# glennhickey/teHmm

Measured on AMD Instinct MI355X. Metric: genome positions/sec (Viterbi+posterior), 35 states x 10 tracks, higher is better.
Workload: dtype f64

## Files before the change

### tehmm_amd/csrc/tehmm_aux.hip.h

```cpp
#pragma once
#include "tehmm_kernels.hip.h"

namespace tehmm {

__global__ __launch_bounds__(256) void k_segment_table(int64_t T, int K, const uint8_t *data, int64_t n_seg,
                                                       const int64_t *off, const uint8_t *is_gauss,
                                                       const double *mapback, uint8_t *out, double *means) {
  __shared__ unsigned hist[4][256];
  const int lane = threadIdx.x & 63, w = threadIdx.x >> 6;
  const int64_t nw = (int64_t)gridDim.x * 4;
  for (int64_t i = (int64_t)blockIdx.x * 4 + w; i < n_seg; i += nw) {
    const int64_t a = off[i], b = i + 1 < n_seg ? off[i + 1] : T;
    for (int k = 0; k < K; ++k) {
      if (is_gauss[k]) {
        if (lane == 0) {
          const double *mb = mapback + (int64_t)k * 256;
          double total = 0.0;
          for (int64_t x = a; x < b; ++x) total += mb[data[x * K + k]];
          means[i * K + k] = total / (double)(b - a);
          out[i * K + k] = data[a * K + k];
        }
        continue;
      }
      unsigned *h = hist[w];
// ... 256 lines not shown
      const int j = kq + 4 * s;
      double v = 0.0;
      if (s < KS && j < N) v = log_domain ? row[j] : (dead ? 0.0 : exp(row[j] - c));
      else if (s < KS && log_domain) v = -INFINITY;
      else if (s == KS) v = (log_domain || dead) ? 0.0 : c;
      o[kq * KSP + s] = v;
    }
  }
}
__global__ void k_pack_ptab_lds(int K, const int *rowbase, const int *rowcnt, const int *ldsbase, int lds_zero,
                                int zero_row, int ROW_D, int ROW_L, const double *ptab, double *ptab_lds) {
  const int k = blockIdx.x;
  int src, dst, cnt;
  if (k == K) { src = zero_row; dst = lds_zero; cnt = 1; }
  else { if (ldsbase[k] < 0) return; src = rowbase[k]; dst = ldsbase[k]; cnt = rowcnt[k]; }
  for (int i = threadIdx.x; i < cnt * ROW_L; i += blockDim.x) {
    const int r = i / ROW_L, c = i - r * ROW_L;
    ptab_lds[(int64_t)(dst + r) * ROW_L + c] = c < ROW_D ? ptab[(int64_t)(src + r) * ROW_D + c] : 0.0;
  }
}

__global__ void k_stats_logprob(int n, const int *ids, const double *fwd_lp, double *stats) {
  if (blockIdx.x == 0 && threadIdx.x == 0) {
    double s = 0.0;
    for (int i = 0; i < n; ++i) s += fwd_lp[ids[i]];
    stats[0] += s;
    stats[1] += (double)n;
  }
}

}
```

### tehmm_amd/csrc/tehmm_fused.hip.h

```cpp
#pragma once
#include "tehmm_lane.hip.h"

namespace tehmm {

template <int NT>
struct FusedGeom {
  static constexpr int KS = NT / 4;
  static constexpr int KSP = ((KS + 1) + 1) & ~1;
  static constexpr int RT = (NT + 15) / 16;
  static constexpr int SLICE_B = KSP * 8;
  static constexpr int ROW_D = 4 * KSP;
  static constexpr int ROW_D_LDS = 4 * KSP + 2;
};

#ifndef TEHMM_FUSED_2W
#define TEHMM_FUSED_2W 36
#endif
#define TEHMM_FUSED_BLKW 24
#ifndef TEHMM_FUSED_NSLOT_CAP
#define TEHMM_FUSED_NSLOT_CAP 64
#endif

struct FusedTab {
  const unsigned long long *rixx;
  const double *ptab;
  const double *ptab_lds;
  int FKW;
  int SB, NB;
  int K, n_glb;
  int lds_rows;
  double normalize;
};

template <int NT>
__device__ __forceinline__ void fused_load_lds(const double *lds, int row, int kq, double (&x)[FusedGeom<NT>::KSP]) {
  using G = FusedGeom<NT>;
  lds_cd2 *p = (lds_cd2 *)(size_t)((unsigned)(size_t)(__attribute__((address_space(3))) const double *)lds +
                                   (unsigned)(row * (G::ROW_D_LDS * 8) + kq * G::SLICE_B));
#pragma unroll
  for (int i = 0; i < G::KSP / 2; ++i) {
    const d2v v = p[i];
    x[2 * i] = v.x;
    x[2 * i + 1] = v.y;
  }
}
template <int NT>
__device__ __forceinline__ void fused_load_glb(const double *tab, int row, int kq, double (&x)[FusedGeom<NT>::KSP]) {
// ... 16 lines not shown
  const auto c = __builtin_amdgcn_permlane16_swap(lo1, lo1, false, false);
  const auto d = __builtin_amdgcn_permlane16_swap(hi1, hi1, false, false);
  return __hiloint2double((int)d[0], (int)c[0]) + __hiloint2double((int)d[1], (int)c[1]);
}
__device__ __forceinline__ double item_max4(double t) {
  const unsigned lo = __double2loint(t), hi = __double2hiint(t);
  const auto a = __builtin_amdgcn_permlane32_swap(lo, lo, false, false);
  const auto b = __builtin_amdgcn_permlane32_swap(hi, hi, false, false);
  const double t1 = fmax(__hiloint2double((int)b[0], (int)a[0]), __hiloint2double((int)b[1], (int)a[1]));
  const unsigned lo1 = __double2loint(t1), hi1 = __double2hiint(t1);
  const auto c = __builtin_amdgcn_permlane16_swap(lo1, lo1, false, false);
  const auto d = __builtin_amdgcn_permlane16_swap(hi1, hi1, false, false);
  return fmax(__hiloint2double((int)d[0], (int)c[0]), __hiloint2double((int)d[1], (int)c[1]));
}

typedef unsigned int fused_u4 __attribute__((ext_vector_type(4)));
struct IndexWindow {
  const fused_u4 *src;
  unsigned lds_base;
  int lane, dir, NB;
  int cur = -1;
  fused_u4 r0, r1, r2;
  bool inflight = false;

  __device__ __forceinline__ void request(int blk) {
    if (blk < 0 || blk >= NB) { inflight = false; return; }
    const fused_u4 *p = src + (int64_t)blk * 192 + lane * 3;
    r0 = p[0];
    r1 = p[1];
    r2 = p[2];
    inflight = true;
  }
  __device__ __forceinline__ void commit(int blk) {
    typedef __attribute__((address_space(3))) fused_u4 lds_u4;
    lds_u4 *d = (lds_u4 *)(size_t)(lds_base + (unsigned)((blk & 1) * 3072 + lane * 48));
    d[0] = r0;
    d[1] = r1;
    d[2] = r2;
    cur = blk;
  }
  __device__ __forceinline__ void start(int blk) {
    request(blk);
    commit(blk);
    request(blk + dir);
  }
  __device__ __forceinline__ void need(int blk) {
    if (blk != cur) {
      commit(blk);
      request(blk + dir);
    }
  }
  __device__ __forceinline__ unsigned word_addr(int blk, int r, int FKW, int w) const {
    return lds_base + (unsigned)((blk & 1) * 3072 + ((r * FKW + w) * 16 + (lane & 15)) * 8);
  }
};
__device__ __forceinline__ unsigned long long lds_read_u64(unsigned addr) {
  typedef __attribute__((address_space(3))) const unsigned long long lds_cu64;
  return *(lds_cu64 *)(size_t)addr;
}

template <int NT, bool LOGDOM>
struct EmisStream {
  using G = FusedGeom<NT>;
  static constexpr int NSLOT = G::KS < TEHMM_FUSED_NSLOT_CAP ? G::KS : TEHMM_FUSED_NSLOT_CAP;
  static constexpr int NGS = NSLOT > 1 ? 2 : 1;
  static constexpr int GF = NSLOT >= 8 ? 4 : NSLOT / 2;
  const FusedTab &ft;
  const double *lds;
  IndexWindow &win;
  const int kq;
  unsigned wbase = 0;
  double q[G::KS];
  double sc = 0.0;
  double xa[G::KSP];
  double xc[G::KSP];
  unsigned long long wcur = 0;

  __device__ __forceinline__ EmisStream(const FusedTab &ft_, const double *lds_, IndexWindow &win_, int kq_)
      : ft(ft_), lds(lds_), win(win_), kq(kq_) {}
  static __device__ __forceinline__ int entry(unsigned long long w, int i) { return (int)((w >> (16 * (i & 3))) & 0xffffull); }
  __device__ __forceinline__ unsigned long long word(int w) const { return lds_read_u64(wbase + (unsigned)w * 128u); }
  __device__ __forceinline__ void fold(const double (&x)[G::KSP]) {
#pragma unroll
    for (int s = 0; s < G::KS; ++s) q[s] = LOGDOM ? q[s] + x[s] : q[s] * x[s];
    if (!LOGDOM) sc += x[G::KS];
  }
  __device__ __forceinline__ void glb_request(int i) { fused_load_glb<NT>(ft.ptab, entry(word(i >> 2), i), kq, xa); }
  __device__ __forceinline__ void begin(int e) {
    const int blk = e / ft.SB, r = e - blk * ft.SB;
    win.need(blk);
    wbase = win.word_addr(blk, r, ft.FKW, 0);
#pragma unroll
    for (int s = 0; s < G::KS; ++s) q[s] = LOGDOM ? 0.0 : 1.0;
    sc = 0.0;
    glb_request(0);
    wcur = word(ft.n_glb >> 2);
  }
  __device__ __forceinline__ void slot(int k) {
    if (k >= NSLOT) return;
    const int il = ft.n_glb + k;
    if (k > 0) fold(xc);
    if (k == GF && NSLOT > 1) {
      fold(xa);
      glb_request(1);
    }
    fused_load_lds<NT>(lds, entry(wcur, il), kq, xc);
    if (k + 1 < NSLOT) wcur = word((il + 1) >> 2);
  }
  __device__ __forceinline__ void finish(int N, double (&qo)[G::KS], double &ms) {
    fold(xc);
    fold(xa);
    for (int i = NGS; i < ft.n_glb; ++i) {
      glb_request(i);
      fold(xa);
    }
    for (int il = ft.n_glb + NSLOT; il < ft.K; ++il) {
      fused_load_lds<NT>(lds, entry(word(il >> 2), il), kq, xc);
      fold(xc);
    }
    if (LOGDOM) {
      double m = -INFINITY;
#pragma unroll
      for (int s = 0; s < G::KS; ++s) {
        q[s] *= ft.normalize;
        m = fmax(m, kq + 4 * s < N ? q[s] : -INFINITY);
      }
      m = item_max4(m);
      const bool good = m > -1e20;
#pragma unroll
      for (int s = 0; s < G::KS; ++s) qo[s] = (good && kq + 4 * s < N) ? exp_nonpos(q[s] - m) : 0.0;
      ms = good ? m : 0.0;
    } else {
#pragma unroll
      for (int s = 0; s < G::KS; ++s) qo[s] = q[s];
      ms = sc;
    }
  }
};

template <int NT>
__host__ __device__ inline size_t fused_lds_bytes(int lds_rows, bool post_tiles) {
  return (size_t)lds_rows * FusedGeom<NT>::ROW_D_LDS * 8 + 4 * 2 * 3072 + (post_tiles ? 4 * (16 * NT * 8 + 128) : 0);
}
template <int NT>
__device__ __forceinline__ void fused_stage(const FusedTab &ft, double *lds) {
  const int n = ft.lds_rows * FusedGeom<NT>::ROW_D_LDS;
  for (int i = threadIdx.x; i < n; i += blockDim.x) lds[i] = ft.ptab_lds[i];
}

struct FusedOrder {
  int K, n_glb, FKW, KP, SB, NB, Wu;
  int zero_glb, zero_lds;
  unsigned char order[TEHMM_MAX_TRACKS];
  int base[TEHMM_MAX_TRACKS];
  int cnt[TEHMM_MAX_TRACKS];
};
__global__ __launch_bounds__(256) void k_fused_rowindex(IntervalTab iv, LaneGeom lg, FusedOrder fo, const uint8_t *obs,
                                                        unsigned long long *rixx) {
  const int E = fo.NB * fo.SB;
  const int64_t n = (int64_t)lg.n_groups * 4 * E * 16;
  const int per_blk = 16 * fo.SB;
  for (int64_t idx = blockIdx.x * (int64_t)blockDim.x + threadIdx.x; idx < n; idx += (int64_t)gridDim.x * blockDim.x) {
    const int64_t tb = idx / per_blk;
    const int rem = (int)(idx - tb * per_blk);
    const int i16 = rem / fo.SB;
    const int e = (int)(tb % fo.NB) * fo.SB + (rem - i16 * fo.SB);
    const int64_t tile = tb / fo.NB;
    const int64_t item = tile * 16 + i16;
    const bool valid = item < lg.n_items;
    const int id = valid ? lg.item_iv[item] : 0;
    const int64_t T = iv.len[id];
    int64_t t = (valid ? lg.item_t0[item] : 0) - fo.Wu + e;
    t = t < 0 ? 0 : (t >= T ? T - 1 : t);
    const uint8_t *orow = obs + (iv.pos0[id] + (T > 0 ? t : 0)) * fo.KP;
    const int blk = e / fo.SB, r = e - blk * fo.SB;
    unsigned long long *dst = rixx + ((tile * fo.NB + blk) * TEHMM_FUSED_BLKW + (int64_t)r * fo.FKW) * 16 + i16;
    for (int w = 0; w < fo.FKW; ++w) {
      unsigned long long word = 0;
      for (int b = 0; b < 4; ++b) {
        const int i = 4 * w + b;
        int v = 0;
        if (i < fo.K) {
          const int sym = orow[fo.order[i]];
          v = sym < fo.cnt[i] ? fo.base[i] + sym : (i < fo.n_glb ? fo.zero_glb : fo.zero_lds);
        }
        word |= (unsigned long long)(v & 0xffff) << (16 * b);
      }
      dst[(int64_t)w * 16] = word;
    }
  }
}

template <int NT, bool LOGDOM>
__global__ __launch_bounds__(256) __attribute__((amdgpu_waves_per_eu(NT <= TEHMM_FUSED_2W ? 2 : 1, NT <= TEHMM_FUSED_2W ? 2 : 1)))
void k_fused_fwd(IntervalTab iv, FusedTab ft, LaneGeom lg, int N, int CS, int Wu,
                 const double *__restrict__ tab , float *al32, double *chkf, double *pre,
                 double *end, double *slog32) {
  using G = FusedGeom<NT>;
  constexpr int KS = G::KS, RT = G::RT;
  extern __shared__ double fused_lds[];
  fused_stage<NT>(ft, fused_lds);
  __syncthreads();
  const int lane = threadIdx.x & 63;
  const int tile = blockIdx.x * 4 + (threadIdx.x >> 6);
  if (tile >= lg.n_groups * 4) return;
// ... 14 lines not shown
    for (int s = 0; s < KS; ++s) {
      const int j = 16 * rt + (lane & 15), k = 4 * s + kq;
      tf[rt][s] = (j < NT) ? tab[k * NT + j] : 0.0;
    }
  }
  double v[KS];
#pragma unroll
  for (int s = 0; s < KS; ++s) v[s] = (kq + 4 * s < N) ? 1.0 / (double)N : 0.0;
  double slog = 0.0;
  auto vec_out = [&](double *dst) {
    const int64_t po = ((((item >> 6) * NT) + kq) << 6) + (item & 63);
#pragma unroll
    for (int s = 0; s < KS; ++s) dst[po + ((int64_t)(4 * s) << 6)] = v[s];
  };
  const double qnan = __longlong_as_double(0x7ff8000000000000LL);
  IndexWindow win;
  win.src = (const fused_u4 *)ft.rixx + (int64_t)tile * ft.NB * 192;
  win.lds_base = (unsigned)(size_t)(__attribute__((address_space(3))) const double *)fused_lds +
                 (unsigned)(ft.lds_rows * G::ROW_D_LDS * 8 + (threadIdx.x >> 6) * 2 * 3072);
  win.lane = lane;
  win.dir = 1;
  win.NB = ft.NB;
  win.start(0);
  double q[KS], ms;
  EmisStream<NT, LOGDOM> es(ft, fused_lds, win, kq);
  es.begin(0);
#pragma unroll
  for (int k = 0; k < KS; ++k) es.slot(k);
  es.finish(N, q, ms);
  const int E1 = ft.NB * ft.SB - 1;
  es.begin(min(1, E1));
  {
    float2 *ar = (float2 *)al32 + al32_index<NT>(lg, item, 0, kq) / 2;
#pragma unroll
    for (int p = 0; p < (KS + 1) / 2; ++p) ar[(int64_t)p * 64] = make_float2(0.f, 0.f);
  }
#ifdef TEHMM_STAMPS
// ... 104 lines not shown
    }
  }
  double v[KS];
#pragma unroll
  for (int s = 0; s < KS; ++s) v[s] = 0.0;
  const int64_t prow0 = (iv.out0[id] + t0) * N;
  auto vec_out = [&](double *dst) {
    const int64_t po = ((((item >> 6) * NT) + kq) << 6) + (item & 63);
#pragma unroll
    for (int s = 0; s < KS; ++s) dst[po + ((int64_t)(4 * s) << 6)] = v[s];
  };
  const double eps = 1.1920928955078125e-07;
  const double inv_epsden = 1.0 / (1.0 + (double)N * eps);
  const double qnan = __longlong_as_double(0x7ff8000000000000LL);
  const int top = L + wu - 1;
  IndexWindow win;
  win.src = (const fused_u4 *)ft.rixx + (int64_t)tile * ft.NB * 192;
  win.lds_base = (unsigned)(size_t)(__attribute__((address_space(3))) const double *)fused_lds +
                 (unsigned)(ft.lds_rows * G::ROW_D_LDS * 8 + (threadIdx.x >> 6) * 2 * 3072);
  win.lane = lane;
  win.dir = -1;
  win.NB = ft.NB;
  win.start((L + 2 * Wu - 1) / ft.SB);
  typedef __attribute__((address_space(3))) double lds_f64;
  typedef __attribute__((address_space(3))) long long lds_i64;
  const unsigned ptile = (unsigned)(size_t)(__attribute__((address_space(3))) const double *)fused_lds +
                         (unsigned)(ft.lds_rows * G::ROW_D_LDS * 8 + 4 * 2 * 3072 + (threadIdx.x >> 6) * (16 * NT * 8 + 128));
  const unsigned pinfo = ptile + 16 * NT * 8;
  if (!ESTEP && kq == 0) *(lds_i64 *)(size_t)(pinfo + (lane & 15) * 8) = run ? (long long)prow0 : -1ll;
  double q[KS], ms;
  EmisStream<NT, LOGDOM> es(ft, fused_lds, win, kq);
  es.begin(L + 2 * Wu - 1);
#pragma unroll
  for (int k = 0; k < KS; ++k) es.slot(k);
  es.finish(N, q, ms);
  es.begin(max(L + 2 * Wu - 2, 0));
#ifdef TEHMM_STAMPS
  unsigned long long stq[4] = {0, 0, 0, 0}, stt = stamp_now();
#define FST(i) do { const unsigned long long n_ = stamp_now(); stq[i] += n_ - stt; stt = n_; } while (0)
#else
#define FST(i)
#endif
// ... 141 lines not shown
```

### tehmm_amd/csrc/tehmm_hip.hip

```cpp
#include <climits>
#include "tehmm_kernels.hip.h"
#include "tehmm_coop.hip.h"
#include "tehmm_lane.hip.h"
#include "tehmm_lane3.hip.h"
#include "tehmm_place.hip.h"
#include "tehmm_aux.hip.h"
#include "tehmm_fused.hip.h"
#include "tehmm_estep.hip.h"
#include "tehmm_wide_estep.hip.h"
#include "tehmm_wide.hip.h"
#include "tehmm_large.hip.h"

#include <algorithm>
#include <atomic>
#include <cmath>
#include <cstdio>
#include <cstdlib>
#include <cstring>
#include <mutex>
#include <numeric>
#include <string>
#include <thread>
#include <vector>

// ... 224 lines not shown
  double normalize = 1.0;
  DBuf<double> lt, ltT, A, AT, pi, tab, ltab;
  DBuf<double> ltG, AG, ATG;
  DBuf<float> ltP;
  DBuf<double> ptab, ptab_lds;
  DBuf<int> d_rowinfo;
  int KSP = 0;
  bool large = false;
  uint64_t uid = 0;
  uint64_t version = 0;
  bool ptab_log = false;
  int rowbase[TEHMM_MAX_TRACKS];
  int rowcnt[TEHMM_MAX_TRACKS];
  int ldsbase[TEHMM_MAX_TRACKS];
  int lds_rows = 0, lds_zero = 0;
  std::vector<double> h_lt;
  DBuf<double> qall[2];
  DBuf<int> qok[2];
  uint64_t q_version[2] = {~(uint64_t)0, ~(uint64_t)0};
};

struct EstepWork {
  DBuf<double> alpha, beta, wrows, fwd_lp;
  DBuf<double> statbuf;
  double *C = nullptr, *D = nullptr, *start = nullptr, *stat = nullptr;
  DBuf<int> escale, dead, order, chunk_iv;
  DBuf<int64_t> grow0, chunk_t0;
  int64_t rows_cap = 0;
  int n_cap = 0, N = 0;
  EstepGroups h_groups;
// ... 16 lines not shown

struct LaneWork {
  int L = 0, CS = 0, NP = 0, n_items = 0, n_groups = 0;
  bool no_vlane = false;
  std::vector<int> h_iv;
  std::vector<int64_t> h_t0, h_first;
  int64_t h_first_item(int id) const { return h_first[(size_t)id]; }
  DBuf<int> item_iv, ok_f, ok_b, link_f, link_b, runend_f, runstart_b;
  DBuf<double> glog_f, cpre_f, dl_f, lr_f, dl_b;
  DBuf<int64_t> item_t0, ifirst;
  DBuf<double> B, BH, MS, AL, BE, pre_f, end_f, pre_b, end_b, slog32;
  DBuf<double> chk, chkf;
  DBuf<double> sink;
  DBuf<float> AL32;
  DBuf<float> GAM32, WZ32;
  DBuf<unsigned long long> rix;
  uint64_t rix_model = 0;
  int rix_L = 0, rix_Wu = 0;
  uint64_t wu_model = 0, wu_version = 0;
  int wu_L = 0, wu_val = 0;
  DBuf<int> probe_iv, probe_steps;
  DBuf<int64_t> probe_t0;
  DBuf<double> vpre, vend, vgain, vtierows, vpiecemin, qtabs;
  DBuf<float> B32;
  DBuf<VitChunks> d_vc;
  DBuf<VitItems> d_vi;
  DBuf<int> vbad, vntie, vties, wk_g, wk_e, wk_items;
  DBuf<PlaceCounts> place;
  DBuf<int> gclass;
  VitChunks up_vc{};
  VitItems up_vi{};
  bool up_valid = false;
  int soft_ties = 0;
// ... 259 lines not shown
int tehmm_update_counts_u16(int64_t T, int K, int N, int S, const uint16_t *obs, int n_iv, const int64_t *starts,
                            const int64_t *ends, const int32_t *states, const double *segRatios, double *obsStats) {
  return update_counts_impl<uint16_t>(T, K, N, S, obs, n_iv, starts, ends, states, segRatios, obsStats);
}
int tehmm_update_counts_i32(int64_t T, int K, int N, int S, const int32_t *obs, int n_iv, const int64_t *starts,
                            const int64_t *ends, const int32_t *states, const double *segRatios, double *obsStats) {
  return update_counts_impl<int32_t>(T, K, N, S, obs, n_iv, starts, ends, states, segRatios, obsStats);
}

static int build_ptab(tehmm_model *m) {
  if (m->NP > 64) return TEHMM_OK;
  const int KS = m->NP / 4, KSP = ((KS + 1) + 1) & ~1, ROW_D = 4 * KSP, ROW_L = ROW_D + 2, K = m->K;
  m->KSP = KSP;
  m->ptab_log = m->normalize != 1.0;
  if (!m->ptab.p) {
    HIPCHK(m->ptab.alloc((size_t)(m->R + 1) * ROW_D));
    HIPCHK(m->ptab_lds.alloc((size_t)std::max(1, m->lds_rows) * ROW_L));
    std::vector<int> info((size_t)3 * K);
    for (int k = 0; k < K; ++k) { info[k] = m->rowbase[k]; info[K + k] = m->rowcnt[k]; info[2 * K + k] = m->ldsbase[k]; }
    HIPCHK(m->d_rowinfo.upload(info.data(), info.size()));
  }
  hipLaunchKernelGGL(k_build_ptab, dim3(grid_for(m->R + 1, 64)), dim3(64), 0, 0, m->R + 1, m->N, m->NP, KSP,
                     (const double *)m->tab.p, m->ptab_log ? 1 : 0, m->ptab.p);
  if (m->lds_rows > 0)
    hipLaunchKernelGGL(k_pack_ptab_lds, dim3(K + 1), dim3(256), 0, 0, K, (const int *)m->d_rowinfo.p,
                       (const int *)m->d_rowinfo.p + K, (const int *)m->d_rowinfo.p + 2 * K, m->lds_zero, m->R, ROW_D,
                       ROW_L, (const double *)m->ptab.p, m->ptab_lds.p);
  HIPCHK(hipGetLastError());
  HIPCHK(hipDeviceSynchronize());
  return TEHMM_OK;
}

static int model_create_large(int N, int K, int S, const double *lt, const double *pi, const double *logProbs,
                              double normalize, const int32_t *symbolsPerTrack, tehmm_model_t **out) {
  tehmm_model *m = new tehmm_model();
  {
    static std::atomic<uint64_t> next_uid{1u << 30};
    m->uid = next_uid.fetch_add(1);
  }
  m->N = N;
  m->K = K;
// ... 358 lines not shown
    if (b->sP) (void)hipStreamDestroy(b->sP);
    if (b->sB) (void)hipStreamDestroy(b->sB);
    for (int i = 0; i < 2; ++i)
      if (b->evX[i]) (void)hipEventDestroy(b->evX[i]);
  }
  for (int i = 0; i < 2; ++i)
    if (b->stage[i]) (void)hipHostFree(b->stage[i]);
  delete b;
  return TEHMM_OK;
}

int64_t tehmm_batch_total(const tehmm_batch_t *b) { return b ? b->total : 0; }

int tehmm_batch_reset_cache(tehmm_batch_t *b) {
  if (!b) return fail(TEHMM_ERR_ARG, "tehmm_batch_reset_cache: NULL handle");
  b->lw.rix_model = 0;
  b->lw.rix_L = 0;
  b->lw.rix_Wu = 0;
  b->lw.wu_val = 0;
  return TEHMM_OK;
}

static void fill_tabs(const tehmm_model *m, const tehmm_batch *b, IntervalTab &iv, EmisTab &em,
                      bool emis_ratios) {
  iv.order = b->d_order.p;
  iv.pos0 = b->d_pos0.p;
  iv.len = b->d_len.p;
  iv.out0 = b->d_out0.p;
  iv.n = b->n;
  em.obs32 = (const uint32_t *)b->obs.p;
  em.tab = m->tab.p;
  em.ratios = emis_ratios ? b->ratios.p : nullptr;
  em.normalize = m->normalize;
// ... 661 lines not shown
                     lw.MS.p, lw.BE.p, lw.pre_b.p, lw.end_b.p, (double *)nullptr);
  hipLaunchKernelGGL((k_fb_itemlinks<NT>), gridit, dim3(256), 0, st, lg, m->N, lw.pre_f.p, lw.end_f.p, lw.pre_b.p,
                     lw.end_b.p, lw.dl_f.p, lw.lr_f.p, lw.dl_b.p, 2);
  hipLaunchKernelGGL((k_fb_stitch<NT>), gridc, dim3(256), 0, st, iv, lg, fc, m->N, lw.slog32.p, lw.end_b.p,
                     lw.dl_f.p, lw.lr_f.p, lw.dl_b.p, lw.ok_f.p, lw.ok_b.p, 2);
  hipLaunchKernelGGL(k_fb_runs, gridi, dim3(64), 0, st, iv, fc, (const int *)lw.ok_f.p, (const int *)lw.ok_b.p,
                     2);
  (void)hipEventRecord(ev_mid, st);
  hipLaunchKernelGGL((k_fb_fix<NT, 1, false, true>), dim3(b->n), dim3(128), lds, st, iv, em, fc, m->N, m->A.p,
                     m->lt.p, m->pi.p, (const double *)nullptr, lw.BE.p, b->fwd_lp.p, b->dead.p,
                     (double *)nullptr, (int *)nullptr, 1, b->sw.stats.p, lg, (const int *)lw.ok_b.p);
  (void)hipStreamWaitEvent(st, b->evX[1], 0);
}

template <int NT>
static int fused_prepare(tehmm_batch *b, const tehmm_model *m, const IntervalTab &iv, int Wu, hipStream_t st, FusedOrder &fo) {
  LaneWork &lw = b->lw;
  const LaneGeom lg = lane_geom(lw);
  std::memset(&fo, 0, sizeof(fo));
  fo.K = m->K;
  fo.KP = b->KP;
  fo.Wu = Wu;
  fo.zero_glb = m->R;
  fo.zero_lds = m->lds_zero;
  {
    constexpr int NSLOT = EmisStream<NT, false>::NSLOT, NGS = EmisStream<NT, false>::NGS;
    int slot = 0;
    auto pad = [&]() { fo.order[slot] = 0; fo.base[slot] = 0; fo.cnt[slot] = 0; ++slot; };
    for (int k = 0; k < m->K; ++k)
      if (m->ldsbase[k] < 0) { fo.order[slot] = (unsigned char)k; fo.base[slot] = m->rowbase[k]; fo.cnt[slot] = m->rowcnt[k]; ++slot; }
    while (slot < NGS) pad();
    fo.n_glb = slot;
    for (int k = 0; k < m->K; ++k)
      if (m->ldsbase[k] >= 0) { fo.order[slot] = (unsigned char)k; fo.base[slot] = m->ldsbase[k]; fo.cnt[slot] = m->rowcnt[k]; ++slot; }
    while (slot - fo.n_glb < NSLOT) pad();
    fo.K = slot;
  }
  {
    static const int ok[] = {1, 2, 3, 4, 6, 8, 12, 24};
    int need = (fo.K + 3) / 4;
    fo.FKW = 24;
    for (int d : ok) if (d >= need) { fo.FKW = d; break; }
  }
  fo.SB = TEHMM_FUSED_BLKW / fo.FKW;
  fo.NB = (lw.L + 2 * Wu + fo.SB - 1) / fo.SB;
  if (!lw.rix.p || lw.rix_model != m->uid || lw.rix_L != lw.L || lw.rix_Wu != Wu) {
    const size_t words = (size_t)lw.n_groups * 4 * fo.NB * TEHMM_FUSED_BLKW * 16;
    lw.rix_model = 0;
    HIPCHK(lw.rix.ensure(words + 16));
    hipLaunchKernelGGL(k_fused_rowindex, dim3(grid_for((int64_t)lw.n_groups * 4 * fo.NB * fo.SB * 16, 256, 1 << 20)),
                       dim3(256), 0, st, iv, lg, fo, (const uint8_t *)b->obs.p, lw.rix.p);
    lw.rix_model = m->uid;
    lw.rix_L = lw.L;
    lw.rix_Wu = Wu;
  }
  return TEHMM_OK;
}

template <int NT>
static int launch_fused_fb(tehmm_batch *b, const tehmm_model *m, const IntervalTab &iv, const EmisTab &em_in,
                           const FbChunks &fc, int Wu, hipStream_t st, hipEvent_t ev_fwd, hipEvent_t ev_mid,
                           bool estep = false, int half = 0, hipEvent_t ev_fwdk = nullptr) {
  LaneWork &lw = b->lw;
  const LaneGeom lg = lane_geom(lw);
  const dim3 gridm((unsigned)lw.n_groups);
  const dim3 gridc((fc.n + 255) / 256);
  const dim3 gridit((lw.n_items + 255) / 256);
  const dim3 gridi(std::max(1, b->n));
  FusedOrder fo;
  if (int rcp = fused_prepare<NT>(b, m, iv, Wu, st, fo)) return rcp;
  FusedTab ft;
  ft.rixx = lw.rix.p;
  ft.ptab = m->ptab.p;
  ft.ptab_lds = m->ptab_lds.p;
  ft.FKW = fo.FKW;
  ft.SB = fo.SB;
  ft.NB = fo.NB;
  ft.K = fo.K;
  ft.n_glb = fo.n_glb;
  ft.lds_rows = m->lds_rows;
  ft.normalize = m->normalize;
  const EmisTab emc = b->n > 256 ? without_lds_tables(em_in) : em_in;
  const size_t lds_f = fused_lds_bytes<NT>(m->lds_rows, false), lds_b = fused_lds_bytes<NT>(m->lds_rows, true);
  const size_t lds_c = ((size_t)2 * 64 * (NT + 1) + 2 * 64 + NT + (size_t)emc.lds_rows * NT + 8) * sizeof(double);
  allow_lds(k_fb_fix<NT, 0, false, true, true>, lds_c);
  allow_lds(k_fb_fix<NT, 1, false, true, true>, lds_c);
#define TEHMM_FUSED_LAUNCH(LOG_)                                                                                     \
  do {                                                                                                              \
    allow_lds(k_fused_fwd<NT, LOG_>, lds_f);                                                                         \
    allow_lds(k_fused_bwd<NT, LOG_, true>, lds_b);                                                                   \
    if (half != 2) {                                                                                                \
    hipLaunchKernelGGL((k_fused_fwd<NT, LOG_>), gridm, dim3(256), lds_f, st, iv, ft, lg, m->N, fc.CS, Wu,            \
                       (const double *)m->A.p, lw.AL32.p, lw.chkf.p, lw.pre_f.p, lw.end_f.p, lw.slog32.p);           \
    if (ev_fwdk) (void)hipEventRecord(ev_fwdk, st);                                                                  \
    hipLaunchKernelGGL((k_fb_itemlinks<NT>), gridit, dim3(256), 0, st, lg, m->N, lw.pre_f.p, lw.end_f.p,             \
                       lw.pre_b.p, lw.end_b.p, lw.dl_f.p, lw.lr_f.p, lw.dl_b.p, 1);                                  \
    hipLaunchKernelGGL((k_fb_stitch<NT>), gridc, dim3(256), 0, st, iv, lg, fc, m->N, lw.slog32.p, lw.end_b.p,        \
                       lw.dl_f.p, lw.lr_f.p, lw.dl_b.p, lw.ok_f.p, lw.ok_b.p, 1);                                    \
// ... 746 lines not shown
  p.CS = kn.spec_chunk;
  const bool spec_ok = p.coop && p.CS > 0 && m->NP <= 64 && b->total >= 2 * (int64_t)p.CS;
  p.vspec = p.vit && spec_ok && (!p.ratio || (ratio_lane_ok(m) && m->NP <= TEHMM_RATIO_LANE_MAX));
  p.fspec = p.postr && spec_ok;
  p.fused_fb = kn.fused && m->ptab.p != nullptr && m->K <= 78;
  p.LS = (p.vspec || p.fspec) ? lane_sub_size(p.CS, b->total, kn.lane_sub) : 0;
  return p;
}

static int plan_lanes(EvalPlan &p, const tehmm_model *m, tehmm_batch *b, const EvalKnobs &kn) {
  LaneWork &lw = b->lw;
  if (p.LS > 0 && !lw.AL.p && !lw.AL32.p && !lw.B.p && !lw.B32.p) {
    size_t free_b = 0, total_b = 0;
    HIPCHK(dev_mem_info(&free_b, &total_b));
    const double per = (double)b->total * m->NP * 8.0;
    const double fb_units = p.fspec ? (p.fused_fb ? 0.7 : 3.2) : 0.0, p0_units = (p.vspec && !p.fused_fb) ? 0.5 : 0.0;
    lw.no_vlane = per * (fb_units + p0_units + 1.0) > 0.85 * (double)free_b;
    if (per * (fb_units + p0_units) > 0.85 * (double)free_b) p.LS = 0;
  }
  bool want_vlane = kn.lane_vit;
  if (p.LS > 0 && want_vlane && !lw.no_vlane && !lw.B.p && (lw.AL.p || lw.AL32.p || lw.B32.p)) {
    size_t free_b = 0, total_b = 0;
    HIPCHK(dev_mem_info(&free_b, &total_b));
    if ((double)b->total * m->NP * 8.0 * 1.6 > 0.85 * (double)free_b) lw.no_vlane = true;
  }
  if (lw.no_vlane) want_vlane = false;
  if (p.ratio && p.vspec && !(p.LS > 0 && want_vlane && (p.fused_fb || !(p.fspec && p.LS > 0)))) {
    p.vspec = false;
    if (!p.fspec) p.LS = 0;
  }
  p.vlane = p.vspec && p.LS > 0 && want_vlane;
// ... 542 lines not shown
    vc.ntie = sw.ntie.p; vc.ties = sw.ties.p; vc.tierows = sw.tierows.p; vc.segmin = sw.segmin.p;
    vc.offend = sw.offend.p; vc.clink = sw.clink.p; vc.clk = sw.clk.p;
    vc.rtarget = sw.rtarget.p; vc.rsel = sw.rsel.p; vc.racc = sw.racc.p; vc.rmn = sw.rmn.p;
    vc.tsoft = sw.tsoft.p; vc.tpar = sw.tpar.p;
  }
  if (p.dev_place) {
    rc = eval_place_setup(c);
    if (rc) return rc;
  }
  rc = eval_emis_p0(c);
  if (rc) return rc;
  if (p.postr && p.defer_post) eval_emission(c);
  if (p.split_post) {
    rc = eval_posterior(c, 1);
    if (rc) return rc;
  } else if (p.postr && p.defer_post && p.flane && p.fused_fb) {
    FusedOrder fo_unused;
    nt_dispatch(m->NP, [&](auto nt) { rc = fused_prepare<nt>(b, m, c.iv, c.WuF, b->sP, fo_unused); });
    if (rc) return rc;
  }
  if (p.postr && !p.defer_post) {
    eval_emission(c);
    if (!p.wide_defer) {
      rc = eval_posterior(c, 0);
      if (rc) return rc;
    }
  }
  if (p.vit) {
    rc = eval_viterbi(c);
    if (rc) return rc;
  }
  rc = eval_finish_wide(c);
  if (rc) return rc;
  eval_timings(p, b);
// ... 1123 lines not shown
```

Measured before the change: 1.527 billion.

## Read raw observation bytes in fused kernels instead of precomputed row-index table

Drops the k_fused_rowindex precompute pass and its large 64-bit row-index buffer. The fused forward/backward kernels now stream raw observation bytes into LDS and compute table row indices on the fly from per-track metadata (column, count, base) held in scalar registers. The LDS table gets a per-track zero tail row so out-of-range symbols clamp without a branch. This removes a full extra pass and its memory traffic and shrinks the memory estimate, at the cost of more index arithmetic, byte-wide LDS reads and a slower gather path near interval edges.

```diff
diff --git a/tehmm_amd/csrc/tehmm_aux.hip.h b/tehmm_amd/csrc/tehmm_aux.hip.h
--- a/tehmm_amd/csrc/tehmm_aux.hip.h
+++ b/tehmm_amd/csrc/tehmm_aux.hip.h
@@ -294,9 +294,10 @@
   int src, dst, cnt;
   if (k == K) { src = zero_row; dst = lds_zero; cnt = 1; }
   else { if (ldsbase[k] < 0) return; src = rowbase[k]; dst = ldsbase[k]; cnt = rowcnt[k]; }
-  for (int i = threadIdx.x; i < cnt * ROW_L; i += blockDim.x) {
+  const int tail = k == K ? 0 : 1;
+  for (int i = threadIdx.x; i < (cnt + tail) * ROW_L; i += blockDim.x) {
     const int r = i / ROW_L, c = i - r * ROW_L;
-    ptab_lds[(int64_t)(dst + r) * ROW_L + c] = c < ROW_D ? ptab[(int64_t)(src + r) * ROW_D + c] : 0.0;
+    ptab_lds[(int64_t)(dst + r) * ROW_L + c] = c < ROW_D ? ptab[(int64_t)(r < cnt ? src + r : zero_row) * ROW_D + c] : 0.0;
   }
 }
 
diff --git a/tehmm_amd/csrc/tehmm_fused.hip.h b/tehmm_amd/csrc/tehmm_fused.hip.h
--- a/tehmm_amd/csrc/tehmm_fused.hip.h
+++ b/tehmm_amd/csrc/tehmm_fused.hip.h
@@ -16,21 +16,28 @@
 #ifndef TEHMM_FUSED_2W
 #define TEHMM_FUSED_2W 36
 #endif
-#define TEHMM_FUSED_BLKW 24
+#define TEHMM_FUSED_BLKD 6
+#define TEHMM_FUSED_BLKB (TEHMM_FUSED_BLKD * 256)
+#define TEHMM_FUSED_MAXK 96
 #ifndef TEHMM_FUSED_NSLOT_CAP
 #define TEHMM_FUSED_NSLOT_CAP 64
 #endif
 
 struct FusedTab {
-  const unsigned long long *rixx;
+  const uint8_t *obs;
   const double *ptab;
   const double *ptab_lds;
-  int FKW;
+  int KP;
   int SB, NB;
   int K, n_glb;
   int lds_rows;
+  int zero_glb;
   double normalize;
+  unsigned meta[TEHMM_FUSED_MAXK + 1];
 };
+__host__ __device__ inline unsigned fused_meta(int col, int cnt, int base) {
+  return (unsigned)col | (unsigned)cnt << 7 | (unsigned)base << 16;
+}
 
 template <int NT>
 __device__ __forceinline__ void fused_load_lds(const double *lds, int row, int kq, double (&x)[FusedGeom<NT>::KSP]) {
@@ -77,29 +84,53 @@
   return fmax(__hiloint2double((int)d[0], (int)c[0]), __hiloint2double((int)d[1], (int)c[1]));
 }
 
-typedef unsigned int fused_u4 __attribute__((ext_vector_type(4)));
-struct IndexWindow {
-  const fused_u4 *src;
+struct ObsWindow {
+  const uint8_t *row0;
+  int lo, hi;
   unsigned lds_base;
-  int lane, dir, NB;
+  int lane, dir, NB, SB, KP, Wu;
   int cur = -1;
-  fused_u4 r0, r1, r2;
-  bool inflight = false;
-
+  unsigned r[TEHMM_FUSED_BLKD];
+
+  __device__ __forceinline__ void init(const FusedTab &ft, const IntervalTab &iv, int id, int64_t t0, int64_t T, int Wu_,
+                                       unsigned lds_base_, int lane_, int dir_) {
+    row0 = ft.obs + (T > 0 ? (iv.pos0[id] + t0) * ft.KP : 0);
+    const int64_t big = 1 << 30;
+    lo = T > 0 ? (int)max(-t0, -big) : 0;
+    hi = T > 0 ? (int)min(T - 1 - t0, big) : 0;
+    lds_base = lds_base_;
+    lane = lane_;
+    dir = dir_;
+    NB = ft.NB;
+    SB = ft.SB;
+    KP = ft.KP;
+    Wu = Wu_;
+  }
   __device__ __forceinline__ void request(int blk) {
-    if (blk < 0 || blk >= NB) { inflight = false; return; }
-    const fused_u4 *p = src + (int64_t)blk * 192 + lane * 3;
-    r0 = p[0];
-    r1 = p[1];
-    r2 = p[2];
-    inflight = true;
+    if (blk < 0 || blk >= NB) return;
+    const int KW = KP >> 2;
+    const int rel0 = blk * SB - Wu;
+    int kq = lane >> 4;
+    asm volatile("" : "+v"(kq));
+    if (__all(rel0 >= lo && rel0 + (TEHMM_FUSED_BLKD * 4 - 1) / KW <= hi)) {
+      const unsigned *p = (const unsigned *)(row0 + ((int64_t)rel0 * KP + kq * 4));
+#pragma unroll
+      for (int d = 0; d < TEHMM_FUSED_BLKD; ++d) r[d] = p[d * 4];
+    } else {
+      const int rdiv = 65536 / KW + 1;
+#pragma unroll
+      for (int d = 0; d < TEHMM_FUSED_BLKD; ++d) {
+        const int g = 4 * d + kq, rr = (g * rdiv) >> 16, w = g - rr * KW;
+        const int rel = min(max(rel0 + rr, lo), hi);
+        r[d] = *(const unsigned *)(row0 + ((int64_t)rel * KP + w * 4));
+      }
+    }
   }
   __device__ __forceinline__ void commit(int blk) {
-    typedef __attribute__((address_space(3))) fused_u4 lds_u4;
-    lds_u4 *d = (lds_u4 *)(size_t)(lds_base + (unsigned)((blk & 1) * 3072 + lane * 48));
-    d[0] = r0;
-    d[1] = r1;
-    d[2] = r2;
+    typedef __attribute__((address_space(3))) unsigned lds_u32;
+    lds_u32 *d = (lds_u32 *)(size_t)(lds_base + (unsigned)((blk & 1) * TEHMM_FUSED_BLKB + lane * 4));
+#pragma unroll
+    for (int i = 0; i < TEHMM_FUSED_BLKD; ++i) d[i * 64] = r[i];
     cur = blk;
   }
   __device__ __forceinline__ void start(int blk) {
@@ -113,13 +144,13 @@
       request(blk + dir);
     }
   }
-  __device__ __forceinline__ unsigned word_addr(int blk, int r, int FKW, int w) const {
-    return lds_base + (unsigned)((blk & 1) * 3072 + ((r * FKW + w) * 16 + (lane & 15)) * 8);
+  __device__ __forceinline__ unsigned row_addr(int blk, int r) const {
+    return lds_base + (unsigned)((blk & 1) * TEHMM_FUSED_BLKB + r * (KP >> 2) * 64 + (lane & 15) * 4);
   }
 };
-__device__ __forceinline__ unsigned long long lds_read_u64(unsigned addr) {
-  typedef __attribute__((address_space(3))) const unsigned long long lds_cu64;
-  return *(lds_cu64 *)(size_t)addr;
+__device__ __forceinline__ unsigned lds_read_u8(unsigned addr) {
+  typedef __attribute__((address_space(3))) const unsigned char lds_cu8;
+  return *(lds_cu8 *)(size_t)addr;
 }
 
 template <int NT, bool LOGDOM>
@@ -128,58 +159,99 @@
   static constexpr int NSLOT = G::KS < TEHMM_FUSED_NSLOT_CAP ? G::KS : TEHMM_FUSED_NSLOT_CAP;
   static constexpr int NGS = NSLOT > 1 ? 2 : 1;
   static constexpr int GF = NSLOT >= 8 ? 4 : NSLOT / 2;
+  static constexpr int NSCH = NGS + NSLOT;
   const FusedTab &ft;
   const double *lds;
-  IndexWindow &win;
+  ObsWindow &win;
   const int kq;
   unsigned wbase = 0;
   double q[G::KS];
   double sc = 0.0;
   double xa[G::KSP];
   double xc[G::KSP];
-  unsigned long long wcur = 0;
-
-  __device__ __forceinline__ EmisStream(const FusedTab &ft_, const double *lds_, IndexWindow &win_, int kq_)
-      : ft(ft_), lds(lds_), win(win_), kq(kq_) {}
-  static __device__ __forceinline__ int entry(unsigned long long w, int i) { return (int)((w >> (16 * (i & 3))) & 0xffffull); }
-  __device__ __forceinline__ unsigned long long word(int w) const { return lds_read_u64(wbase + (unsigned)w * 128u); }
+  unsigned scur = 0;
+  unsigned mcol[LOGDOM ? 1 : NSCH], mcnt[LOGDOM ? 1 : NSCH], mbase[LOGDOM ? 1 : NSCH], mw[LOGDOM ? NSCH : 1];
+
+  static __device__ __forceinline__ unsigned col_off(unsigned m) { return ((m & 0x7c) << 4) | (m & 3); }
+  static __device__ __forceinline__ unsigned cnt_of(unsigned m) { return (m >> 7) & 0x1ff; }
+  static __device__ __forceinline__ unsigned base_of(unsigned m) { return m >> 16; }
+  __device__ __forceinline__ EmisStream(const FusedTab &ft_, const double *lds_, ObsWindow &win_, int kq_)
+      : ft(ft_), lds(lds_), win(win_), kq(kq_) {
+#pragma unroll
+    for (int i = 0; i < NSCH; ++i) {
+      const unsigned m = ft.meta[i < NGS ? i : ft.n_glb + (i - NGS)];
+      if constexpr (LOGDOM) {
+        mw[i] = m;
+        asm volatile("" : "+s"(mw[i]));
+      } else {
+        mcol[i] = col_off(m);
+        mcnt[i] = cnt_of(m);
+        mbase[i] = base_of(m);
+        asm volatile("" : "+s"(mcol[i]), "+s"(mcnt[i]), "+s"(mbase[i]));
+      }
+    }
+  }
+  __device__ __forceinline__ unsigned word_of(int i) const {
+    unsigned w = mw[LOGDOM ? i : 0];
+    asm volatile("" : "+s"(w));
+    return w;
+  }
+  __device__ __forceinline__ unsigned col_at(int i) const { if constexpr (LOGDOM) return col_off(word_of(i)); else return mcol[i]; }
+  __device__ __forceinline__ unsigned cnt_at(int i) const { if constexpr (LOGDOM) return cnt_of(word_of(i)); else return mcnt[i]; }
+  __device__ __forceinline__ unsigned base_at(int i) const { if constexpr (LOGDOM) return base_of(word_of(i)); else return mbase[i]; }
+  __device__ __forceinline__ unsigned sym_at(unsigned coff) const { return lds_read_u8(wbase + coff); }
+  static __device__ __forceinline__ int row_lds(unsigned sym, unsigned cnt, unsigned base) { return (int)(min(sym, cnt) + base); }
+  __device__ __forceinline__ int row_glb(unsigned sym, unsigned cnt, unsigned base) const {
+    return sym < cnt ? (int)(sym + base) : ft.zero_glb;
+  }
   __device__ __forceinline__ void fold(const double (&x)[G::KSP]) {
 #pragma unroll
     for (int s = 0; s < G::KS; ++s) q[s] = LOGDOM ? q[s] + x[s] : q[s] * x[s];
     if (!LOGDOM) sc += x[G::KS];
   }
-  __device__ __forceinline__ void glb_request(int i) { fused_load_glb<NT>(ft.ptab, entry(word(i >> 2), i), kq, xa); }
+  __device__ __forceinline__ void glb_request(int i) {
+    fused_load_glb<NT>(ft.ptab, row_glb(sym_at(col_at(i)), cnt_at(i), base_at(i)), kq, xa);
+  }
   __device__ __forceinline__ void begin(int e) {
     const int blk = e / ft.SB, r = e - blk * ft.SB;
     win.need(blk);
-    wbase = win.word_addr(blk, r, ft.FKW, 0);
+    wbase = win.row_addr(blk, r);
 #pragma unroll
     for (int s = 0; s < G::KS; ++s) q[s] = LOGDOM ? 0.0 : 1.0;
     sc = 0.0;
     glb_request(0);
-    wcur = word(ft.n_glb >> 2);
+    scur = sym_at(col_at(NGS));
   }
   __device__ __forceinline__ void slot(int k) {
     if (k >= NSLOT) return;
-    const int il = ft.n_glb + k;
     if (k > 0) fold(xc);
     if (k == GF && NSLOT > 1) {
       fold(xa);
       glb_request(1);
     }
-    fused_load_lds<NT>(lds, entry(wcur, il), kq, xc);
-    if (k + 1 < NSLOT) wcur = word((il + 1) >> 2);
+    fused_load_lds<NT>(lds, row_lds(scur, cnt_at(NGS + k), base_at(NGS + k)), kq, xc);
+    if (k + 1 < NSLOT) scur = sym_at(col_at(NGS + k + 1));
   }
   __device__ __forceinline__ void finish(int N, double (&qo)[G::KS], double &ms) {
     fold(xc);
     fold(xa);
-    for (int i = NGS; i < ft.n_glb; ++i) {
-      glb_request(i);
-      fold(xa);
-    }
-    for (int il = ft.n_glb + NSLOT; il < ft.K; ++il) {
-      fused_load_lds<NT>(lds, entry(word(il >> 2), il), kq, xc);
-      fold(xc);
+    if (NGS < ft.n_glb) {
+      unsigned m = ft.meta[NGS];
+      for (int i = NGS; i < ft.n_glb; ++i) {
+        const unsigned mn = ft.meta[i + 1];
+        fused_load_glb<NT>(ft.ptab, row_glb(sym_at(col_off(m)), cnt_of(m), base_of(m)), kq, xa);
+        fold(xa);
+        m = mn;
+      }
+    }
+    if (ft.n_glb + NSLOT < ft.K) {
+      unsigned m = ft.meta[ft.n_glb + NSLOT];
+      for (int il = ft.n_glb + NSLOT; il < ft.K; ++il) {
+        const unsigned mn = ft.meta[il + 1];
+        fused_load_lds<NT>(lds, row_lds(sym_at(col_off(m)), cnt_of(m), base_of(m)), kq, xc);
+        fold(xc);
+        m = mn;
+      }
     }
     if (LOGDOM) {
       double m = -INFINITY;
@@ -203,55 +275,12 @@
 
 template <int NT>
 __host__ __device__ inline size_t fused_lds_bytes(int lds_rows, bool post_tiles) {
-  return (size_t)lds_rows * FusedGeom<NT>::ROW_D_LDS * 8 + 4 * 2 * 3072 + (post_tiles ? 4 * (16 * NT * 8 + 128) : 0);
+  return (size_t)lds_rows * FusedGeom<NT>::ROW_D_LDS * 8 + 4 * 2 * TEHMM_FUSED_BLKB + (post_tiles ? 4 * (16 * NT * 8 + 128) : 0);
 }
 template <int NT>
 __device__ __forceinline__ void fused_stage(const FusedTab &ft, double *lds) {
   const int n = ft.lds_rows * FusedGeom<NT>::ROW_D_LDS;
   for (int i = threadIdx.x; i < n; i += blockDim.x) lds[i] = ft.ptab_lds[i];
-}
-
-struct FusedOrder {
-  int K, n_glb, FKW, KP, SB, NB, Wu;
-  int zero_glb, zero_lds;
-  unsigned char order[TEHMM_MAX_TRACKS];
-  int base[TEHMM_MAX_TRACKS];
-  int cnt[TEHMM_MAX_TRACKS];
-};
-__global__ __launch_bounds__(256) void k_fused_rowindex(IntervalTab iv, LaneGeom lg, FusedOrder fo, const uint8_t *obs,
-                                                        unsigned long long *rixx) {
-  const int E = fo.NB * fo.SB;
-  const int64_t n = (int64_t)lg.n_groups * 4 * E * 16;
-  const int per_blk = 16 * fo.SB;
-  for (int64_t idx = blockIdx.x * (int64_t)blockDim.x + threadIdx.x; idx < n; idx += (int64_t)gridDim.x * blockDim.x) {
-    const int64_t tb = idx / per_blk;
-    const int rem = (int)(idx - tb * per_blk);
-    const int i16 = rem / fo.SB;
-    const int e = (int)(tb % fo.NB) * fo.SB + (rem - i16 * fo.SB);
-    const int64_t tile = tb / fo.NB;
-    const int64_t item = tile * 16 + i16;
-    const bool valid = item < lg.n_items;
-    const int id = valid ? lg.item_iv[item] : 0;
-    const int64_t T = iv.len[id];
-    int64_t t = (valid ? lg.item_t0[item] : 0) - fo.Wu + e;
-    t = t < 0 ? 0 : (t >= T ? T - 1 : t);
-    const uint8_t *orow = obs + (iv.pos0[id] + (T > 0 ? t : 0)) * fo.KP;
-    const int blk = e / fo.SB, r = e - blk * fo.SB;
-    unsigned long long *dst = rixx + ((tile * fo.NB + blk) * TEHMM_FUSED_BLKW + (int64_t)r * fo.FKW) * 16 + i16;
-    for (int w = 0; w < fo.FKW; ++w) {
-      unsigned long long word = 0;
-      for (int b = 0; b < 4; ++b) {
-        const int i = 4 * w + b;
-        int v = 0;
-        if (i < fo.K) {
-          const int sym = orow[fo.order[i]];
-          v = sym < fo.cnt[i] ? fo.base[i] + sym : (i < fo.n_glb ? fo.zero_glb : fo.zero_lds);
-        }
-        word |= (unsigned long long)(v & 0xffff) << (16 * b);
-      }
-      dst[(int64_t)w * 16] = word;
-    }
-  }
 }
 
 template <int NT, bool LOGDOM>
@@ -296,13 +325,11 @@
     for (int s = 0; s < KS; ++s) dst[po + ((int64_t)(4 * s) << 6)] = v[s];
   };
   const double qnan = __longlong_as_double(0x7ff8000000000000LL);
-  IndexWindow win;
-  win.src = (const fused_u4 *)ft.rixx + (int64_t)tile * ft.NB * 192;
-  win.lds_base = (unsigned)(size_t)(__attribute__((address_space(3))) const double *)fused_lds +
-                 (unsigned)(ft.lds_rows * G::ROW_D_LDS * 8 + (threadIdx.x >> 6) * 2 * 3072);
-  win.lane = lane;
-  win.dir = 1;
-  win.NB = ft.NB;
+  ObsWindow win;
+  win.init(ft, iv, id, t0, T, Wu,
+           (unsigned)(size_t)(__attribute__((address_space(3))) const double *)fused_lds +
+               (unsigned)(ft.lds_rows * G::ROW_D_LDS * 8 + (threadIdx.x >> 6) * 2 * TEHMM_FUSED_BLKB),
+           lane, 1);
   win.start(0);
   double q[KS], ms;
   EmisStream<NT, LOGDOM> es(ft, fused_lds, win, kq);
@@ -437,18 +464,16 @@
   const double inv_epsden = 1.0 / (1.0 + (double)N * eps);
   const double qnan = __longlong_as_double(0x7ff8000000000000LL);
   const int top = L + wu - 1;
-  IndexWindow win;
-  win.src = (const fused_u4 *)ft.rixx + (int64_t)tile * ft.NB * 192;
-  win.lds_base = (unsigned)(size_t)(__attribute__((address_space(3))) const double *)fused_lds +
-                 (unsigned)(ft.lds_rows * G::ROW_D_LDS * 8 + (threadIdx.x >> 6) * 2 * 3072);
-  win.lane = lane;
-  win.dir = -1;
-  win.NB = ft.NB;
+  ObsWindow win;
+  win.init(ft, iv, id, t0, T, Wu,
+           (unsigned)(size_t)(__attribute__((address_space(3))) const double *)fused_lds +
+               (unsigned)(ft.lds_rows * G::ROW_D_LDS * 8 + (threadIdx.x >> 6) * 2 * TEHMM_FUSED_BLKB),
+           lane, -1);
   win.start((L + 2 * Wu - 1) / ft.SB);
   typedef __attribute__((address_space(3))) double lds_f64;
   typedef __attribute__((address_space(3))) long long lds_i64;
   const unsigned ptile = (unsigned)(size_t)(__attribute__((address_space(3))) const double *)fused_lds +
-                         (unsigned)(ft.lds_rows * G::ROW_D_LDS * 8 + 4 * 2 * 3072 + (threadIdx.x >> 6) * (16 * NT * 8 + 128));
+                         (unsigned)(ft.lds_rows * G::ROW_D_LDS * 8 + 4 * 2 * TEHMM_FUSED_BLKB + (threadIdx.x >> 6) * (16 * NT * 8 + 128));
   const unsigned pinfo = ptile + 16 * NT * 8;
   if (!ESTEP && kq == 0) *(lds_i64 *)(size_t)(pinfo + (lane & 15) * 8) = run ? (long long)prow0 : -1ll;
   double q[KS], ms;
diff --git a/tehmm_amd/csrc/tehmm_hip.hip b/tehmm_amd/csrc/tehmm_hip.hip
--- a/tehmm_amd/csrc/tehmm_hip.hip
+++ b/tehmm_amd/csrc/tehmm_hip.hip
@@ -262,6 +262,8 @@
   int rowcnt[TEHMM_MAX_TRACKS];
   int ldsbase[TEHMM_MAX_TRACKS];
   int lds_rows = 0, lds_zero = 0;
+  int pldsbase[TEHMM_MAX_TRACKS];
+  int plds_rows = 0, plds_zero = 0;
   std::vector<double> h_lt;
   DBuf<double> qall[2];
   DBuf<int> qok[2];
@@ -308,9 +310,6 @@
   DBuf<double> sink;
   DBuf<float> AL32;
   DBuf<float> GAM32, WZ32;
-  DBuf<unsigned long long> rix;
-  uint64_t rix_model = 0;
-  int rix_L = 0, rix_Wu = 0;
   uint64_t wu_model = 0, wu_version = 0;
   int wu_L = 0, wu_val = 0;
   DBuf<int> probe_iv, probe_steps;
@@ -600,17 +599,26 @@
   m->KSP = KSP;
   m->ptab_log = m->normalize != 1.0;
   if (!m->ptab.p) {
+    {
+      std::vector<int> ord;
+      for (int k = 0; k < K; ++k) { m->pldsbase[k] = -1; if (m->ldsbase[k] >= 0) ord.push_back(k); }
+      std::sort(ord.begin(), ord.end(), [&](int a, int b) { return m->ldsbase[a] < m->ldsbase[b]; });
+      int used = 0;
+      for (int k : ord) { m->pldsbase[k] = used; used += m->rowcnt[k] + 1; }
+      m->plds_zero = used;
+      m->plds_rows = used + 1;
+    }
     HIPCHK(m->ptab.alloc((size_t)(m->R + 1) * ROW_D));
-    HIPCHK(m->ptab_lds.alloc((size_t)std::max(1, m->lds_rows) * ROW_L));
+    HIPCHK(m->ptab_lds.alloc((size_t)m->plds_rows * ROW_L));
     std::vector<int> info((size_t)3 * K);
-    for (int k = 0; k < K; ++k) { info[k] = m->rowbase[k]; info[K + k] = m->rowcnt[k]; info[2 * K + k] = m->ldsbase[k]; }
+    for (int k = 0; k < K; ++k) { info[k] = m->rowbase[k]; info[K + k] = m->rowcnt[k]; info[2 * K + k] = m->pldsbase[k]; }
     HIPCHK(m->d_rowinfo.upload(info.data(), info.size()));
   }
   hipLaunchKernelGGL(k_build_ptab, dim3(grid_for(m->R + 1, 64)), dim3(64), 0, 0, m->R + 1, m->N, m->NP, KSP,
                      (const double *)m->tab.p, m->ptab_log ? 1 : 0, m->ptab.p);
-  if (m->lds_rows > 0)
+  if (m->plds_rows > 0)
     hipLaunchKernelGGL(k_pack_ptab_lds, dim3(K + 1), dim3(256), 0, 0, K, (const int *)m->d_rowinfo.p,
-                       (const int *)m->d_rowinfo.p + K, (const int *)m->d_rowinfo.p + 2 * K, m->lds_zero, m->R, ROW_D,
+                       (const int *)m->d_rowinfo.p + K, (const int *)m->d_rowinfo.p + 2 * K, m->plds_zero, m->R, ROW_D,
                        ROW_L, (const double *)m->ptab.p, m->ptab_lds.p);
   HIPCHK(hipGetLastError());
   HIPCHK(hipDeviceSynchronize());
@@ -999,9 +1007,6 @@
 
 int tehmm_batch_reset_cache(tehmm_batch_t *b) {
   if (!b) return fail(TEHMM_ERR_ARG, "tehmm_batch_reset_cache: NULL handle");
-  b->lw.rix_model = 0;
-  b->lw.rix_L = 0;
-  b->lw.rix_Wu = 0;
   b->lw.wu_val = 0;
   return TEHMM_OK;
 }
@@ -1693,47 +1698,28 @@
 }
 
 template <int NT>
-static int fused_prepare(tehmm_batch *b, const tehmm_model *m, const IntervalTab &iv, int Wu, hipStream_t st, FusedOrder &fo) {
-  LaneWork &lw = b->lw;
-  const LaneGeom lg = lane_geom(lw);
-  std::memset(&fo, 0, sizeof(fo));
-  fo.K = m->K;
-  fo.KP = b->KP;
-  fo.Wu = Wu;
-  fo.zero_glb = m->R;
-  fo.zero_lds = m->lds_zero;
-  {
-    constexpr int NSLOT = EmisStream<NT, false>::NSLOT, NGS = EmisStream<NT, false>::NGS;
-    int slot = 0;
-    auto pad = [&]() { fo.order[slot] = 0; fo.base[slot] = 0; fo.cnt[slot] = 0; ++slot; };
-    for (int k = 0; k < m->K; ++k)
-      if (m->ldsbase[k] < 0) { fo.order[slot] = (unsigned char)k; fo.base[slot] = m->rowbase[k]; fo.cnt[slot] = m->rowcnt[k]; ++slot; }
-    while (slot < NGS) pad();
-    fo.n_glb = slot;
-    for (int k = 0; k < m->K; ++k)
-      if (m->ldsbase[k] >= 0) { fo.order[slot] = (unsigned char)k; fo.base[slot] = m->ldsbase[k]; fo.cnt[slot] = m->rowcnt[k]; ++slot; }
-    while (slot - fo.n_glb < NSLOT) pad();
-    fo.K = slot;
-  }
-  {
-    static const int ok[] = {1, 2, 3, 4, 6, 8, 12, 24};
-    int need = (fo.K + 3) / 4;
-    fo.FKW = 24;
-    for (int d : ok) if (d >= need) { fo.FKW = d; break; }
-  }
-  fo.SB = TEHMM_FUSED_BLKW / fo.FKW;
-  fo.NB = (lw.L + 2 * Wu + fo.SB - 1) / fo.SB;
-  if (!lw.rix.p || lw.rix_model != m->uid || lw.rix_L != lw.L || lw.rix_Wu != Wu) {
-    const size_t words = (size_t)lw.n_groups * 4 * fo.NB * TEHMM_FUSED_BLKW * 16;
-    lw.rix_model = 0;
-    HIPCHK(lw.rix.ensure(words + 16));
-    hipLaunchKernelGGL(k_fused_rowindex, dim3(grid_for((int64_t)lw.n_groups * 4 * fo.NB * fo.SB * 16, 256, 1 << 20)),
-                       dim3(256), 0, st, iv, lg, fo, (const uint8_t *)b->obs.p, lw.rix.p);
-    lw.rix_model = m->uid;
-    lw.rix_L = lw.L;
-    lw.rix_Wu = Wu;
-  }
-  return TEHMM_OK;
+static void fused_tab(const tehmm_batch *b, const tehmm_model *m, int Wu, FusedTab &ft) {
+  const LaneWork &lw = b->lw;
+  std::memset(&ft, 0, sizeof(ft));
+  ft.obs = (const uint8_t *)b->obs.p;
+  ft.ptab = m->ptab.p;
+  ft.ptab_lds = m->ptab_lds.p;
+  ft.KP = b->KP;
+  ft.lds_rows = m->plds_rows;
+  ft.zero_glb = m->R;
+  ft.normalize = m->normalize;
+  constexpr int NSLOT = EmisStream<NT, false>::NSLOT, NGS = EmisStream<NT, false>::NGS;
+  int slot = 0;
+  for (int k = 0; k < m->K; ++k)
+    if (m->ldsbase[k] < 0) ft.meta[slot++] = fused_meta(k, m->rowcnt[k], m->rowbase[k]);
+  while (slot < NGS) ft.meta[slot++] = fused_meta(0, 0, m->R);
+  ft.n_glb = slot;
+  for (int k = 0; k < m->K; ++k)
+    if (m->ldsbase[k] >= 0) ft.meta[slot++] = fused_meta(k, m->rowcnt[k], m->pldsbase[k]);
+  while (slot - ft.n_glb < NSLOT) ft.meta[slot++] = fused_meta(0, 0, m->plds_zero);
+  ft.K = slot;
+  ft.SB = std::max(1, 4 * TEHMM_FUSED_BLKD / (ft.KP / 4));
+  ft.NB = (lw.L + 2 * Wu + ft.SB - 1) / ft.SB;
 }
 
 template <int NT>
@@ -1746,21 +1732,10 @@
   const dim3 gridc((fc.n + 255) / 256);
   const dim3 gridit((lw.n_items + 255) / 256);
   const dim3 gridi(std::max(1, b->n));
-  FusedOrder fo;
-  if (int rcp = fused_prepare<NT>(b, m, iv, Wu, st, fo)) return rcp;
   FusedTab ft;
-  ft.rixx = lw.rix.p;
-  ft.ptab = m->ptab.p;
-  ft.ptab_lds = m->ptab_lds.p;
-  ft.FKW = fo.FKW;
-  ft.SB = fo.SB;
-  ft.NB = fo.NB;
-  ft.K = fo.K;
-  ft.n_glb = fo.n_glb;
-  ft.lds_rows = m->lds_rows;
-  ft.normalize = m->normalize;
+  fused_tab<NT>(b, m, Wu, ft);
   const EmisTab emc = b->n > 256 ? without_lds_tables(em_in) : em_in;
-  const size_t lds_f = fused_lds_bytes<NT>(m->lds_rows, false), lds_b = fused_lds_bytes<NT>(m->lds_rows, true);
+  const size_t lds_f = fused_lds_bytes<NT>(m->plds_rows, false), lds_b = fused_lds_bytes<NT>(m->plds_rows, true);
   const size_t lds_c = ((size_t)2 * 64 * (NT + 1) + 2 * 64 + NT + (size_t)emc.lds_rows * NT + 8) * sizeof(double);
   allow_lds(k_fb_fix<NT, 0, false, true, true>, lds_c);
   allow_lds(k_fb_fix<NT, 1, false, true, true>, lds_c);
@@ -2537,7 +2512,7 @@
     size_t free_b = 0, total_b = 0;
     HIPCHK(dev_mem_info(&free_b, &total_b));
     const double per = (double)b->total * m->NP * 8.0;
-    const double fb_units = p.fspec ? (p.fused_fb ? 0.7 : 3.2) : 0.0, p0_units = (p.vspec && !p.fused_fb) ? 0.5 : 0.0;
+    const double fb_units = p.fspec ? (p.fused_fb ? 0.57 : 3.2) : 0.0, p0_units = (p.vspec && !p.fused_fb) ? 0.5 : 0.0;
     lw.no_vlane = per * (fb_units + p0_units + 1.0) > 0.85 * (double)free_b;
     if (per * (fb_units + p0_units) > 0.85 * (double)free_b) p.LS = 0;
   }
@@ -3110,10 +3085,6 @@
   if (p.split_post) {
     rc = eval_posterior(c, 1);
     if (rc) return rc;
-  } else if (p.postr && p.defer_post && p.flane && p.fused_fb) {
-    FusedOrder fo_unused;
-    nt_dispatch(m->NP, [&](auto nt) { rc = fused_prepare<nt>(b, m, c.iv, c.WuF, b->sP, fo_unused); });
-    if (rc) return rc;
   }
   if (p.postr && !p.defer_post) {
     eval_emission(c);
```

New measurement: 1.537 billion (median of 6 runs). Within noise of the previous version (+0.7%).
